# vmingchen/PacBioAssembly

Hardware: AMD Instinct MI355X
Metric: aligned candidate pairs/sec (whole node), 15 kb PacBio reads @15% error (higher is better)
Workload: dtype u32

## Files before the change

### pacbioassembly_amd/csrc/align_bitvec.h

```cpp
#ifndef PBA_ALIGN_BITVEC_H
#define PBA_ALIGN_BITVEC_H

#include <limits.h>

#include <type_traits>

#include "align_rowsweep.h"
#include "dev_common.h"
#include "eq_table.h"
#include "text_ring.h"

#ifndef PBA_BV_EQTAB
#define PBA_BV_EQTAB 1
#endif
#ifndef PBA_BV_RING
#define PBA_BV_RING 1
#endif
#define PBA_BV_EQTAB_NB(nb) (PBA_BV_EQTAB && PBA_BV_RING && (nb) <= 2)

#define PBA_BV_MAX_NB 8
#define PBA_BV_FIN_WORDS(nb) ((2 * (nb) + 1) * 64)
#define PBA_BV_LDS_BYTES(nb) (PBA_BV_EQTAB_NB(nb) ? eqt_lds_words(nb) * 4 : PBA_BV_FIN_WORDS(nb) * 4 + PBA_TXR_BYTES)
#define PBA_BV_BAND_NUM 9
#define PBA_BV_BAND_DEN 16

__device__ __host__ inline int bv_max_span(int nb) { return 2016 * nb + 64; }
__device__ __host__ inline int bv_nb_for_span(int span) {
    const int need = (span - 64 + 2015) / 2016;
    const int nb = need < 1 ? 1 : need;
    return nb <= 4 ? nb : (nb <= 6 ? 6 : (nb <= 8 ? 8 : 0));
}
__device__ __host__ inline int bv_nb_for(int w) { return bv_nb_for_span(2 * w); }

__device__ __forceinline__ uint64_t load_bases32(const uint8_t *seq, int idx) {
    const uint8_t *p = seq + (idx >> 2);
    const uint64_t hi = __builtin_bswap64(ld_u64(p)), nx = __builtin_bswap64(ld_u64(p + 8));
    const int sh = 2 * (idx & 3);
    return sh ? (hi << sh) | (nx >> (64 - sh)) : hi;
}

__device__ __forceinline__ uint32_t compress_even64(uint64_t x) {
    uint32_t lo = (uint32_t)x & 0x55555555u, hi = (uint32_t)(x >> 32) & 0x55555555u;
    lo = (lo | (lo >> 1)) & 0x33333333u; hi = (hi | (hi >> 1)) & 0x33333333u;
    lo = (lo | (lo >> 2)) & 0x0F0F0F0Fu; hi = (hi | (hi >> 2)) & 0x0F0F0F0Fu;
    lo = (lo | (lo >> 4)) & 0x00FF00FFu; hi = (hi | (hi >> 4)) & 0x00FF00FFu;
    lo = (lo | (lo >> 8)) & 0x0000FFFFu; hi = (hi | (hi >> 8)) & 0x0000FFFFu;
    return lo | (hi << 16);
}

__device__ __forceinline__ void load_planes32(const PackedFetch &f, int e, uint32_t &plo, uint32_t &phi) {
    const int idx = f.dir > 0 ? f.org + e : f.org - e - 31;
    const uint32_t *p = f.pl + 2 * (ptrdiff_t)(idx >> 5);
    const uint32_t sh = (uint32_t)idx & 31u;
    const uint32_t lo = __builtin_amdgcn_alignbit(p[2], p[0], sh);
    const uint32_t hi = __builtin_amdgcn_alignbit(p[3], p[1], sh);
    plo = f.dir > 0 ? lo : __builtin_bitreverse32(lo);
    phi = f.dir > 0 ? hi : __builtin_bitreverse32(hi);
}

__device__ __forceinline__ void planes_from_packed(const uint8_t *seq, int idx, uint32_t &plo, uint32_t &phi) {
    const uint64_t x = load_bases32(seq, idx);
    plo = __builtin_bitreverse32(compress_even64(x));
    phi = __builtin_bitreverse32(compress_even64(x >> 1));
}

__device__ __forceinline__ uint32_t addc_mask(uint32_t a, uint32_t b, uint64_t cin, uint64_t &cout) {
    uint32_t d;
    asm("v_addc_co_u32 %0, %1, %2, %3, %4" : "=v"(d), "=s"(cout) : "v"(a), "v"(b), "s"(cin));
    return d;
}

__device__ __forceinline__ uint32_t or_of_and(uint32_t a, uint32_t b, uint32_t c) {
    uint32_t d;
    asm("v_bitop3_b32 %0, %1, %2, %3 bitop3:0xf8" : "=v"(d) : "v"(a), "v"(b), "v"(c));
    return d;
}
__device__ __forceinline__ uint32_t or_of_and_s(uint32_t a, uint32_t b, uint32_t c) {
    uint32_t d;
    asm("v_bitop3_b32 %0, %1, %2, %3 bitop3:0xf8" : "=v"(d) : "v"(a), "v"(b), "s"(c));
    return d;
}
__device__ __forceinline__ uint32_t eq_mask(uint32_t a, uint32_t b, uint32_t c) {
    uint32_t d;
    asm("v_bitop3_b32 %0, %1, %2, %3 bitop3:0x09" : "=v"(d) : "v"(a), "v"(b), "v"(c));
    return d;
}
__device__ __forceinline__ uint64_t bv_uniform64(uint64_t x) {
    return (uint64_t)(uint32_t)__builtin_amdgcn_readfirstlane((int)(uint32_t)x) |
           (uint64_t)(uint32_t)__builtin_amdgcn_readfirstlane((int)(uint32_t)(x >> 32)) << 32;
}
__device__ __forceinline__ uint64_t bv_orn2(uint64_t a, uint64_t b) {
    uint64_t d;
    asm("s_orn2_b64 %0, %1, %2" : "=s"(d) : "s"(a), "s"(b) : "scc");
    return d;
}
__device__ __forceinline__ uint64_t bv_and2(uint64_t a, uint64_t b) {
    uint64_t d;
    asm("s_and_b64 %0, %1, %2" : "=s"(d) : "s"(a), "s"(b) : "scc");
    return d;
}
__device__ __forceinline__ uint32_t bit_mask(uint32_t x, int k) {
    uint32_t d;
    asm("v_bfe_i32 %0, %1, %2, 1" : "=v"(d) : "v"(x), "s"(k));
    return d;
}

#define PBA_BV_CK_WORDS(nb) ((nb) * 128 + 128)
#define PBA_BV_BAIL 0x40000000
template <int NB>
__device__ __forceinline__ void bv_ckpt_store(uint32_t *tr, int tb, int lane, const uint32_t *Pv, const uint32_t *Mv, int s_cur,
                                              uint32_t opened, uint64_t hp_last, uint64_t hn_last) {
    uint32_t *ck = tr + (size_t)((tb - 1) >> 5) * PBA_BV_CK_WORDS(NB);
#pragma unroll
    for (int nb = 0; nb < NB; ++nb) { ck[nb * 128 + lane] = Pv[nb]; ck[nb * 128 + 64 + lane] = Mv[nb]; }
    ck[NB * 128 + lane] = (uint32_t)s_cur | (opened << 31);
    if (lane < 4)
        ck[NB * 128 + 64 + lane] = lane == 0 ? (uint32_t)hp_last : lane == 1 ? (uint32_t)(hp_last >> 32) : lane == 2 ? (uint32_t)hn_last : (uint32_t)(hn_last >> 32);
}

template <int NB, int TRACE = 0, bool BAIL = false, bool RING = false>
__device__ __forceinline__ int bitvec_pass(const PackedFetch &rowsF, int nr, const PackedFetch &colsF, int m, int wleft, int w,
                                           double R, int &best_out, int &besti_out, int &diag_out, uint32_t *fin,
                                           uint32_t *tr = nullptr, bool swap_roles = false, int bail_w = 0) {
    constexpr int RB = 32 * NB;
    const int lane = threadIdx.x & (PBA_WAVE - 1);
    m = __builtin_amdgcn_readfirstlane(m); nr = __builtin_amdgcn_readfirstlane(nr);
    w = __builtin_amdgcn_readfirstlane(w); wleft = __builtin_amdgcn_readfirstlane(wleft);
    const int S = (nr + RB - 1) / RB;
    const int s_m = (m - 1) / RB;
    const int nb_m = ((m - 1) - s_m * RB) >> 5, r_m = (m - 1) & 31;
    const int t1 = m + s_m;
    const int t_end = m + S - 1;
    (void)nb_m; (void)r_m;

    constexpr bool EQT = RING && PBA_BV_EQTAB_NB(NB);
    constexpr int FIN_SB = EQT ? PBA_EQT_LETTERS * NB * PBA_EQT_LANES + PBA_TXR_SLOTS : 2 * NB * PBA_WAVE;
    typedef __attribute__((address_space(3))) uint32_t lds_u32;
    lds_u32 *const tab_lane = (lds_u32 *)fin + lane;
    (void)tab_lane;
#define PBA_BV_FILL_ROWS(sb)                                                          \
    _Pragma("unroll") for (int nb = 0; nb < NB; ++nb) {                               \
        uint32_t plo_, phi_;                                                          \
        load_planes32(rowsF, (sb) * RB + 32 * nb, plo_, phi_);                        \
        tab_lane[(0 * NB + nb) * PBA_EQT_LANES] = ~(plo_ | phi_);                     \
        tab_lane[(1 * NB + nb) * PBA_EQT_LANES] = plo_ & ~phi_;                       \
        tab_lane[(2 * NB + nb) * PBA_EQT_LANES] = ~plo_ & phi_;                       \
        tab_lane[(3 * NB + nb) * PBA_EQT_LANES] = plo_ & phi_;                        \
    }

    uint32_t Pv[NB], Mv[NB], Plo[NB], Phi[NB], acc[NB];
    int s_cur = lane;
    uint32_t opened = 0;
    (void)opened; (void)Plo; (void)Phi;
    if (s_cur < S) {
        if constexpr (EQT) { PBA_BV_FILL_ROWS(s_cur) } else {
#pragma unroll
        for (int nb = 0; nb < NB; ++nb) load_planes32(rowsF, s_cur * RB + 32 * nb, Plo[nb], Phi[nb]);
        }
    }
#pragma unroll
    for (int nb = 0; nb < NB; ++nb) { Pv[nb] = ~0u; Mv[nb] = 0u; acc[nb] = 0u; }

    int T_open = 1, s_op = 0;
    int T_close = min(m, RB + w) + 1, s_cl = 0;
    int T_diag = 1, s_dg = 0;
    int T_seg = min(32, m) + 1, s_sg = 0;
    int s_next = 1;
    (void)T_diag; (void)s_dg;
    constexpr bool LANE_SB = !RING;
#define PBA_BV_LANE_SB() (LANE_SB ? s_cur : s_cl + ((lane - s_cl) & (PBA_WAVE - 1)))
#define PBA_BV_LANE_OPEN() (LANE_SB ? opened != 0 : PBA_BV_LANE_SB() < s_op)
    constexpr bool DIAG_FOLD = !BAIL && NB != 6;
    constexpr int OH_SH = DIAG_FOLD ? 32 : 0;
    typedef typename std::conditional<DIAG_FOLD, uint64_t, uint32_t>::type onehot_t;
    onehot_t one = DIAG_FOLD ? (onehot_t)1 << OH_SH : 0;
    int qd = 0;
    constexpr bool LANE_HOT = BAIL;
    uint32_t dmw = 0;
    (void)dmw; (void)one; (void)qd;

    uint32_t wl = 0, wh = 0;
    typedef __attribute__((address_space(3))) typename std::conditional<EQT, uint32_t, uint64_t>::type txr_cell;
    txr_cell *const ring = (txr_cell *)(fin + (EQT ? PBA_EQT_LETTERS * NB * PBA_EQT_LANES : PBA_BV_FIN_WORDS(NB)));
    const txr_cell *ta = ring;
    (void)wl; (void)wh; (void)ring; (void)ta;
    if constexpr (EQT) {
        static_assert(PBA_TXR_SLOTS <= 3 * PBA_WAVE && PBA_TXR_SLOTS > 2 * PBA_WAVE, "three cells per lane cover the ring");
        ring[lane] = 0; ring[PBA_WAVE + lane] = 0;
        if (lane < PBA_TXR_SLOTS - 2 * PBA_WAVE) ring[2 * PBA_WAVE + lane] = 0;
    }
    int score = 0, fail_row = 0;
    fin[FIN_SB + lane] = 0xFFFFFFFFu;
    uint64_t hp_last = ~0ull, hn_last = 0ull;
    uint64_t live = (S >= PBA_WAVE ? ~0ull : (1ull << S) - 1ull) >> 1;
    uint64_t hpm = ~0ull, hnm = 0ull;

    auto load_text = [&](int tb) {
        if constexpr (RING) {
            const int first = txr_fetch_first(tb, s_cl);
            uint32_t plo, phi;
            load_planes32(colsF, first, plo, phi);
            const int c = lane & (PBA_TXR_CHUNK - 1), slot = txr_slot(first + c), mir = txr_mirror(slot);
            const int dst = (lane >= PBA_TXR_CHUNK && mir >= 0) ? mir : slot;
            if constexpr (EQT) ring[dst] = (((plo >> c) & 1u) | (((phi >> c) & 1u) << 1)) * (uint32_t)(NB * PBA_EQT_LANES * 4);
            else ring[dst] = (uint64_t)(0u - ((plo >> c) & 1u)) | ((uint64_t)(0u - ((phi >> c) & 1u)) << 32);
            ta = ring + txr_addr(tb, PBA_BV_LANE_SB());
        } else {
            load_planes32(colsF, tb - PBA_BV_LANE_SB() - 1, wl, wh);
        }
    };

    auto segment_done = [&](int s, int i) -> int {
        const int rr = i - 1 - s * RB, cnt = (rr & 31) + 1, i0 = i - cnt, q = rr >> 5;
        const int L = s & (PBA_WAVE - 1);
        uint32_t dw = 0;
#pragma unroll
        for (int nb = 0; nb < NB; ++nb) if (q == nb) dw = __builtin_amdgcn_readlane(acc[nb], L);
        dw &= 0xFFFFFFFFu >> (32 - cnt);
        const int end = score + cnt - __builtin_popcount(dw);
        const int ifirst = max(i0 + 1, 11);
        int fr = 0;
        if (i >= ifirst && (double)end > (double)ifirst * R) {
#pragma clang loop unroll(disable) vectorize(disable) interleave(disable)
            for (int k = ifirst - i0; k <= cnt; ++k) {
                const int d = score + k - __builtin_popcount(dw & (0xFFFFFFFFu >> (32 - k)));
                if ((double)d > (double)(i0 + k) * R) { fr = i0 + k; break; }
            }
        }
        if constexpr (BAIL) {
            if (bail_w > 0 && i >= 1024 && fr == 0 &&
                ((float)end - 4.0f * __builtin_sqrtf((float)end)) * (float)m > (float)i * (float)bail_w) fr = PBA_BV_BAIL;
        }
        score = end;
        const bool leaves = rr == RB - 1 && i != m;
        if (lane == L || (DIAG_FOLD && leaves && lane == ((s + 1) & (PBA_WAVE - 1)))) {
#pragma unroll
            for (int nb = 0; nb < NB; ++nb) acc[nb] = 0;
            if constexpr (LANE_HOT) dmw = (i == m || rr == RB - 1) ? 0u : 1u;
        }
        if constexpr (DIAG_FOLD) one = i == m ? 0 : (onehot_t)1 << (leaves ? OH_SH - 1 : OH_SH);
        else one = (i == m || rr == RB - 1) ? 0u : 1u;
        qd = (q + 1) % NB;
        return fr;
    };

#define PBA_BV_EVENTS(DIAG)                                                           \
    {                                                                                 \
        if (DIAG && t == T_seg) {                                                     \
            const int s = s_sg, i = t - 1 - s;                                        \
            seg_fail = segment_done(s, i);                                            \
            if (i == m) T_seg = INT_MAX;                                              \
            else { s_sg = s + (i == s * RB + RB ? 1 : 0); T_seg = min(i + 32, m) + s_sg + 1; } \
        }                                                                             \
        if (t == T_close) {                                                           \
            const int s = s_cl;                                                       \
            if (lane == (s & (PBA_WAVE - 1))) {                                       \
                if (s >= s_m) {               \
                    fin[FIN_SB + lane] = (uint32_t)(LANE_SB ? s_cur : s);  \
                    _Pragma("unroll") for (int nb = 0; nb < NB; ++nb) { fin[2 * nb * PBA_WAVE + lane] = Pv[nb]; fin[(2 * nb + 1) * PBA_WAVE + lane] = Mv[nb]; } \
                }                                                                     \
                                    \
                if constexpr (LANE_SB) { s_cur += PBA_WAVE; opened = 0; }             \
                const int sn = LANE_SB ? s_cur : s + PBA_WAVE;                        \
                 \
                if (s + PBA_WAVE < S) {                                               \
                    if constexpr (EQT) { PBA_BV_FILL_ROWS(sn) } else {                \
                    _Pragma("unroll") for (int nb = 0; nb < NB; ++nb) load_planes32(rowsF, sn * RB + 32 * nb, Plo[nb], Phi[nb]); \
                    }                                                                 \
                }                                                                     \
                if constexpr (RING) ta = ring + txr_addr(t, sn);       \
                else load_text(t - ((t - 1) & 31));                                   \
            }                                                                         \
              \
            if (s + PBA_WAVE < S) {                                                   \
                live |= 1ull << ((s - 1) & (PBA_WAVE - 1));                           \
                hpm = bv_orn2(hp_last, live); hnm = bv_and2(hn_last, live);           \
            }                                                                         \
            live &= ~(1ull << (s & (PBA_WAVE - 1)));                                  \
            s_cl = s + 1;                                                             \
            T_close = s_cl < S ? min(m, s_cl * RB + RB + w) + s_cl + 1 : INT_MAX;     \
        }                                                                             \
        if (t == T_open) {                                                            \
            if (lane == (s_op & (PBA_WAVE - 1))) {                                    \
                _Pragma("unroll") for (int nb = 0; nb < NB; ++nb) { Pv[nb] = ~0u; Mv[nb] = 0u; } \
                if constexpr (LANE_SB) opened = 1;                                    \
            }                                                                         \
            s_op += 1;                                                                \
            T_open = s_op < S ? max(1, s_op * RB + 1 - wleft) + s_op : INT_MAX;       \
        }                                                                             \
        if constexpr (!DIAG_FOLD) {                                                   \
            if (DIAG && t == T_diag) {                                                \
                if (lane == (s_dg & (PBA_WAVE - 1))) {                                \
                    _Pragma("unroll") for (int nb = 0; nb < NB; ++nb) acc[nb] = 0;    \
                    if constexpr (LANE_HOT) dmw = 1u;                                 \
                }                                                                     \
                one = 1u; qd = 0;                                                     \
                s_dg += 1;                                                            \
                T_diag = s_dg * RB < m ? s_dg * (RB + 1) + 1 : INT_MAX;               \
            }                                                                         \
        }                                                                             \
        s_next = min(T_open, T_close);                                                \
        if (DIAG) s_next = min(s_next, DIAG_FOLD ? T_seg : min(T_seg, T_diag));       \
        if constexpr (TRACE == 1) st_on = ((__builtin_amdgcn_ballot_w64(PBA_BV_LANE_OPEN()) >> (lane & 48)) & 0xFFFFull) != 0; \
    }

#define PBA_BV_HIN()                                                                  \
    uint64_t hp = (hpm << 1) | (hpm >> 63);                                           \
    uint64_t hn = (hnm << 1) | (hnm >> 63);
#define PBA_BV_HOUT()                                                                 \
    hp_last = hp; hn_last = hn;                                                       \
    hpm = bv_orn2(hp, live); hnm = bv_and2(hn, live);

#define PBA_BV_BLOCK(nb, PH_PRE, MH_PRE, D0, EQ)                                     \
    {                                                                                \
        const uint32_t Eq = EQT ? eqr[nb] : eq_mask(Plo[nb] ^ clo, Phi[nb], chi);    \
        EQ = Eq;                                                                     \
        const uint32_t pv = Pv[nb], mv = Mv[nb];                                     \
        uint64_t unused;                                                             \
        const uint32_t sum = addc_mask(Eq & pv, pv, hn, unused);    \
        const uint32_t Xh = (sum ^ pv) | Eq;                                         \
        const uint32_t Ph = mv | ~(Xh | pv);                                         \
        const uint32_t Mh = pv & Xh;                                                 \
        D0 = Xh | mv;                                                                \
        PH_PRE = Ph; MH_PRE = Mh;                                                    \
        const uint32_t Ph2 = addc_mask(Ph, Ph, hp, hp);                              \
        const uint32_t Mh2 = addc_mask(Mh, Mh, hn, hn);                              \
        Pv[nb] = Mh2 | ~(D0 | Ph2);                                                  \
        Mv[nb] = Ph2 & D0;                                                           \
    }

    uint2 *const tr_lane = (uint2 *)tr + lane;
    (void)tr_lane;
    bool st_on = false;
    (void)st_on;
#define PBA_BV_TRP() (tr_lane + (size_t)(t - 1) * (NB * 64))
#define PBA_BV_TEXT(OFS)                                                             \
        uint32_t clo = 0, chi = 0, eqr[NB];                                          \
        _Pragma("unroll") for (int nb = 0; nb < NB; ++nb) eqr[nb] = eqn[OFS][nb];    \
        (void)clo; (void)chi; (void)eqr;                                             \
        if constexpr (EQT) { }                                                       \
        else if constexpr (RING) { const uint64_t cell = ta[OFS]; clo = (uint32_t)cell; chi = (uint32_t)(cell >> 32); } \
        else { clo = bit_mask(wl, k + (OFS)); chi = bit_mask(wh, k + (OFS)); }
#define PBA_BV_ROWS(OFS)                                                             \
        {                                                                            \
        const lds_u32 *const row = (const lds_u32 *)((const __attribute__((address_space(3))) uint8_t *)tab_lane + cq[OFS]); \
        _Pragma("unroll") for (int nb = 0; nb < NB; ++nb) eqn[OFS][nb] = row[nb * PBA_EQT_LANES]; \
        }
#define PBA_BV_STEP1(QD, OFS)                                                        \
        {                                                                            \
        const int t = tb + k + (OFS);                                                \
        (void)t;                                                                     \
        PBA_BV_TEXT(OFS)                                                             \
        PBA_BV_HIN();                                                                \
        _Pragma("unroll")                                                            \
        for (int nb = 0; nb < NB; ++nb) {                                            \
            uint32_t d0, php, mhp, eq;                                               \
            PBA_BV_BLOCK(nb, php, mhp, d0, eq);                                      \
            (void)php; (void)mhp; (void)eq;                                          \
            if constexpr (TRACE == 1) {       \
                if (st_on)                    \
                    PBA_BV_TRP()[nb * 64] = make_uint2(eq | ~d0, swap_roles ? Pv[nb] : php); \
            }                                                                        \
                               \
            if constexpr (LANE_HOT) acc[nb] = or_of_and(acc[nb], d0, dmw); else       \
            if ((QD) < 0 || nb == (QD)) acc[nb] = or_of_and_s(acc[nb], d0, (uint32_t)(oh >> OH_SH)); \
        }                                                                            \
        PBA_BV_HOUT()                                                                \
                                               \
        if constexpr (LANE_HOT) asm("v_add_u32 %0, %1, %1" : "=v"(dmw) : "v"(dmw)); else oh <<= 1; \
        }
#define PBA_BV_STRETCH1(QD)                                                          \
        uint32_t cq[2] = {0u, 0u}, eqn[2][NB] = {};                                  \
        (void)cq; (void)eqn;                                                         \
        if constexpr (EQT) {                                                         \
            if ((kstop - k) & 1) { cq[0] = ta[0]; PBA_BV_ROWS(0) PBA_BV_STEP1(QD, 0) ta += 1; k += 1; } \
            while (k < kstop) {                                                      \
                cq[0] = ta[0]; cq[1] = ta[1];                                        \
                PBA_BV_ROWS(0) PBA_BV_ROWS(1)                                        \
                PBA_BV_STEP1(QD, 0)                                                  \
                _Pragma("unroll") for (int nb = 0; nb < NB; ++nb) asm("" : "+v"(Pv[nb]), "+v"(Mv[nb])); \
                PBA_BV_STEP1(QD, 1)                                                  \
                ta += 2; k += 2;                                                     \
            }                                                                        \
        } else if constexpr (RING) {                                                 \
            if ((kstop - k) & 1) { PBA_BV_STEP1(QD, 0) ta += 1; k += 1; }            \
            while (k < kstop) {                                                      \
                PBA_BV_STEP1(QD, 0)                                                  \
                 \
                _Pragma("unroll") for (int nb = 0; nb < NB; ++nb) asm("" : "+v"(Pv[nb]), "+v"(Mv[nb])); \
                PBA_BV_STEP1(QD, 1)                                                  \
                ta += 2; k += 2;                                                     \
            }                                                                        \
        } else {                                                                     \
            do { PBA_BV_STEP1(QD, 0) } while (++k < kstop);                          \
        }
    for (int tbv = 1; tbv <= t1; tbv += 32) {
        const int tb = __builtin_amdgcn_readfirstlane(tbv);
        if constexpr (TRACE == 2) bv_ckpt_store<NB>(tr, tb, lane, Pv, Mv, PBA_BV_LANE_SB(), LANE_SB ? opened : (PBA_BV_LANE_OPEN() ? 1u : 0u), hp_last, hn_last);
        load_text(tb);
        if (fail_row) break;
        int kend = min(32, t1 - tb + 1);
        for (int k = 0; k < kend;) {
        if (tb + k == s_next) {
            const int t = tb + k;
            int seg_fail = 0;
            PBA_BV_EVENTS(true);
            if (seg_fail) { fail_row = seg_fail; kend = k + 1; }
        }
        const int kstop = min(kend, s_next - tb);
        onehot_t oh = 0;
        if constexpr (DIAG_FOLD) oh = (onehot_t)bv_uniform64(one);
        else if constexpr (!LANE_HOT) oh = __builtin_amdgcn_readfirstlane(one);
        if constexpr (NB == 2 && TRACE != 1 && !LANE_HOT) {
            if (__builtin_amdgcn_readfirstlane(qd) == 0) { PBA_BV_STRETCH1(0); } else { PBA_BV_STRETCH1(1); }
        } else {
            PBA_BV_STRETCH1(NB == 1 ? 0 : -1);
        }
        if constexpr (!LANE_HOT) one = oh;
        }
    }
    if (fail_row == 0) fail_row = segment_done(s_m, m);
    if (fail_row) return __builtin_amdgcn_readfirstlane(fail_row);
    s_next = min(T_open, T_close);
    hpm = bv_orn2(hp_last, live); hnm = bv_and2(hn_last, live);

    for (int tb = t1 + 1; tb <= t_end;) {
        const int k0 = (tb - 1) & 31;
        if (k0 == 0) {
            if constexpr (TRACE == 2) bv_ckpt_store<NB>(tr, tb, lane, Pv, Mv, PBA_BV_LANE_SB(), LANE_SB ? opened : (PBA_BV_LANE_OPEN() ? 1u : 0u), hp_last, hn_last);
            load_text(tb);
        }
        const int kend = min(32, k0 + (t_end - tb + 1));
        const int tc = tb - k0;
        for (int k = k0; k < kend;) {
        if (tc + k == s_next) {
            const int t = tc + k;
            int seg_fail = 0;
            (void)seg_fail;
            PBA_BV_EVENTS(false);
        }
        const int kstop = min(kend, s_next - tc);
        do {
        const int t = tc + k;
        (void)t;
        uint32_t cq[1] = {0u}, eqn[1][NB] = {};
        (void)cq; (void)eqn;
        if constexpr (EQT) { cq[0] = ta[0]; PBA_BV_ROWS(0) }
        PBA_BV_TEXT(0)
        PBA_BV_HIN();
#pragma unroll
        for (int nb = 0; nb < NB; ++nb) {
            uint32_t d0, php, mhp, eq;
            PBA_BV_BLOCK(nb, php, mhp, d0, eq);
            (void)d0; (void)eq; (void)php; (void)mhp;
            if constexpr (TRACE == 1) {
                if (st_on)
                    PBA_BV_TRP()[nb * 64] = make_uint2(eq | ~d0, swap_roles ? Pv[nb] : php);
            }
        }
        PBA_BV_HOUT()
        if constexpr (RING) ta += 1;
        } while (++k < kstop);
        }
        tb += kend - k0;
    }
#undef PBA_BV_STRETCH1
#undef PBA_BV_STEP1
#undef PBA_BV_ROWS
#undef PBA_BV_TEXT
#undef PBA_BV_FILL_ROWS
#undef PBA_BV_BLOCK
#undef PBA_BV_TRP
#undef PBA_BV_HOUT
#undef PBA_BV_HIN
#undef PBA_BV_EVENTS
    if (const int sb = PBA_BV_LANE_SB(); PBA_BV_LANE_OPEN() && sb >= s_m && sb < S) {
        fin[FIN_SB + lane] = (uint32_t)sb;
#pragma unroll
        for (int nb = 0; nb < NB; ++nb) { fin[2 * nb * PBA_WAVE + lane] = Pv[nb]; fin[(2 * nb + 1) * PBA_WAVE + lane] = Mv[nb]; }
    }
#undef PBA_BV_LANE_OPEN
#undef PBA_BV_LANE_SB
    const int fin_s = (int)fin[FIN_SB + lane];
    int b_tot[NB], b_min[NB], b_pos[NB];
#pragma unroll
    for (int nb = 0; nb < NB; ++nb) {
        const int row0 = fin_s * RB + nb * 32;
        const uint32_t fpv = fin_s >= 0 ? fin[2 * nb * PBA_WAVE + lane] : 0u, fmv = fin_s >= 0 ? fin[(2 * nb + 1) * PBA_WAVE + lane] : 0u;
        int v = 0, pm = INT_MAX, pp = 0;
        for (int r = 0; r < 32; ++r) {
            const int row = row0 + r + 1;
            if (fin_s >= 0 && row > m && row <= nr) {
                v += (int)((fpv >> r) & 1u) - (int)((fmv >> r) & 1u);
                if (v < pm) { pm = v; pp = r; }
            }
        }
        b_tot[nb] = v; b_min[nb] = pm; b_pos[nb] = pp;
    }
    int gbest = __builtin_amdgcn_readfirstlane(score), gi = m, run = gbest;
    diag_out = gbest;
    for (int sb = s_m; sb < S; ++sb) {
        const int L = sb & (PBA_WAVE - 1);
#pragma unroll
        for (int nb = 0; nb < NB; ++nb) {
            const int pm = __builtin_amdgcn_readlane(b_min[nb], L);
            if (pm != INT_MAX && run + pm < gbest) {
                gbest = run + pm;
                gi = sb * RB + nb * 32 + __builtin_amdgcn_readlane(b_pos[nb], L) + 1;
            }
            run += __builtin_amdgcn_readlane(b_tot[nb], L);
        }
    }
    best_out = gbest;
    besti_out = gi;
    return 0;
}

__device__ __host__ inline int bv_full_wl(int md) { return md / 2 + 1 < md ? md / 2 + 1 : md; }
__device__ __host__ inline bool bitvec_supports(int max_dst) { return bv_nb_for_span(bv_full_wl(max_dst) + max_dst) != 0; }
__device__ __host__ inline int bv_first_w(int md) {
    const int w = (md / 2 > (int)((long long)md * PBA_BV_BAND_NUM / PBA_BV_BAND_DEN)
                       ? md / 2 : (int)((long long)md * PBA_BV_BAND_NUM / PBA_BV_BAND_DEN)) + 1;
    return w > md ? md : w;
}
__device__ __host__ inline int bv_first_wl(int md) {
    const int wl = bv_first_w(md) / 2 + 1;
    return wl > md ? md : wl;
}
__device__ __host__ inline int bv_pass1_w(int md, int nb) {
    int w = bv_first_w(md);
    const int room = (bv_max_span(nb) - 4) * 2 / 3;
    if (room > w) w = room;
    return w > md ? md : w;
}
__device__ __host__ inline int bv_pass1_wl(int md, int nb) {
    const int wl = bv_pass1_w(md, nb) / 2 + 1;
    return wl > md ? md : wl;
}
__device__ __forceinline__ bool bv_fail_certified(int fr, double R, int wl, int md) {
    return 2 * wl + 2 > md || (double)fr * R < (double)(2 * wl + 2);
}
__device__ __forceinline__ bool bv_goal_certified(int best, int wl, int w, int md) {
    return (w >= md && 2 * wl + 1 >= md) || (best <= w && best <= 2 * wl + 1);
}

#define PBA_RC_UNCERTIFIED (-3)

#ifndef PBA_BV_RING
#define PBA_BV_RING 1
#endif
template <int NB, bool BAIL = false>
__device__ __forceinline__ void align_bitvec(const PackedFetch &fa, int la, const PackedFetch &fb, int lb, double R,
                                             int maxn, int maxm, bool full_band, uint16_t *lds, int lds_cells,
                                             AlnOut &o, bool need_diag = false) {
    aln_params(la, lb, R, o);
    const int len_a = o.len_a, len_b = o.len_b, md = o.max_dst;
    if (maxn > 0 && (len_a >= maxn + maxm || md >= maxm)) return;
    const bool a_rows = len_a > len_b;
    const int m = a_rows ? len_b : len_a, n = a_rows ? len_a : len_b;
    if (m <= 10) {
        align_rowsweep(fa, la, fb, lb, R, maxn, maxm, lds, lds_cells, o);
        return;
    }
    const int w = full_band ? md : bv_pass1_w(md, NB), wl = full_band ? bv_full_wl(md) : bv_pass1_wl(md, NB);
    if (wl + w > bv_max_span(NB)) { o.rc = -2; return; }
    const PackedFetch rowsF = a_rows ? fa : fb, colsF = a_rows ? fb : fa;
    int best = 0, besti = 0, diag = 0;
    const int bail_w = (BAIL && !full_band && w < md) ? w : 0;
    const int fr = bitvec_pass<NB, 0, BAIL, PBA_BV_RING && !BAIL>(rowsF, min(n, m + w), colsF, m, w, wl, R, best, besti, diag, (uint32_t *)lds, nullptr, false, bail_w);
    if (fr) {
        bool gave_up = false;
        if constexpr (BAIL) gave_up = fr == PBA_BV_BAIL;
        if (!gave_up && bv_fail_certified(fr, R, wl, md)) o.fail_row = fr; else o.rc = PBA_RC_UNCERTIFIED;
        return;
    }
    if (!bv_goal_certified(best, wl, w, md)) { o.rc = PBA_RC_UNCERTIFIED; return; }
    const bool diag_ok = bv_goal_certified(diag, wl, w, md);
    if (need_diag && !diag_ok) { o.rc = PBA_RC_UNCERTIFIED; return; }
    o.cost = best;
    o.diag = diag_ok ? diag : -1;
    o.matlen_a = a_rows ? besti : m;
    o.matlen_b = a_rows ? m : besti;
    o.rc = ((double)o.matlen_b < (double)len_b * (1.0 - R)) ? -1 : o.matlen_b;
}

#endif
```

Baseline: 20.19 million.

## Shift band state down one lane on segment close instead of rotating lanes

For the EQ-table ring path, closing a segment now shifts Pv/Mv/acc down one lane with DPP, so lane 0 always holds the oldest open segment. This removes the live-mask orn/and work and the rotate in the per-column horizontal carry, which becomes a plain scalar shift. The cost is a special non-rotated step on close columns, DPP moves on every close, and column-indexed LDS addressing. The new mapping touches event handling, the ring addressing and the final readout, so it carries correctness risk.

```diff
diff --git a/pacbioassembly_amd/csrc/align_bitvec.h b/pacbioassembly_amd/csrc/align_bitvec.h
--- a/pacbioassembly_amd/csrc/align_bitvec.h
+++ b/pacbioassembly_amd/csrc/align_bitvec.h
@@ -8,6 +8,7 @@
 #include "align_rowsweep.h"
 #include "dev_common.h"
 #include "eq_table.h"
+#include "lane_shift.h"
 #include "text_ring.h"
 
 #ifndef PBA_BV_EQTAB
@@ -17,6 +18,9 @@
 #define PBA_BV_RING 1
 #endif
 #define PBA_BV_EQTAB_NB(nb) (PBA_BV_EQTAB && PBA_BV_RING && (nb) <= 2)
+#ifndef PBA_BV_SHIFT
+#define PBA_BV_SHIFT 1
+#endif
 
 #define PBA_BV_MAX_NB 8
 #define PBA_BV_FIN_WORDS(nb) ((2 * (nb) + 1) * 64)
@@ -98,6 +102,19 @@
     uint64_t d;
     asm("s_and_b64 %0, %1, %2" : "=s"(d) : "s"(a), "s"(b) : "scc");
     return d;
+}
+__device__ __forceinline__ uint64_t bv_shl1(uint64_t a) {
+    uint64_t d;
+    asm("s_lshl_b64 %0, %1, 1" : "=s"(d) : "s"(a) : "scc");
+    return d;
+}
+__device__ __forceinline__ uint64_t bv_shl1_or1(uint64_t a) {
+    uint64_t d;
+    asm("s_lshl_b64 %0, %1, 1\n\ts_or_b64 %0, %0, 1" : "=&s"(d) : "s"(a) : "scc");
+    return d;
+}
+__device__ __forceinline__ uint32_t bv_lane_below(uint32_t x) {
+    return (uint32_t)__builtin_amdgcn_update_dpp((int)x, (int)x, 0x130 , 0xf, 0xf, false);
 }
 __device__ __forceinline__ uint32_t bit_mask(uint32_t x, int k) {
     uint32_t d;
@@ -136,8 +153,8 @@
     constexpr bool EQT = RING && PBA_BV_EQTAB_NB(NB);
     constexpr int FIN_SB = EQT ? PBA_EQT_LETTERS * NB * PBA_EQT_LANES + PBA_TXR_SLOTS : 2 * NB * PBA_WAVE;
     typedef __attribute__((address_space(3))) uint32_t lds_u32;
-    lds_u32 *const tab_lane = (lds_u32 *)fin + lane;
-    (void)tab_lane;
+    constexpr bool SHIFT = EQT && PBA_BV_SHIFT;
+#define tab_lane ((lds_u32 *)fin + (SHIFT ? lsh_col(lane, s_cl) : lane))
 #define PBA_BV_FILL_ROWS(sb)                                                          \
     _Pragma("unroll") for (int nb = 0; nb < NB; ++nb) {                               \
         uint32_t plo_, phi_;                                                          \
@@ -153,6 +170,8 @@
     uint32_t opened = 0;
     (void)opened; (void)Plo; (void)Phi;
     if (s_cur < S) {
+        constexpr int s_cl = 0;
+        (void)s_cl;
         if constexpr (EQT) { PBA_BV_FILL_ROWS(s_cur) } else {
 #pragma unroll
         for (int nb = 0; nb < NB; ++nb) load_planes32(rowsF, s_cur * RB + 32 * nb, Plo[nb], Phi[nb]);
@@ -168,7 +187,8 @@
     int s_next = 1;
     (void)T_diag; (void)s_dg;
     constexpr bool LANE_SB = !RING;
-#define PBA_BV_LANE_SB() (LANE_SB ? s_cur : s_cl + ((lane - s_cl) & (PBA_WAVE - 1)))
+#define PBA_BV_LANE_SB() (LANE_SB ? s_cur : SHIFT ? lsh_sb(lane, s_cl) : s_cl + ((lane - s_cl) & (PBA_WAVE - 1)))
+#define PBA_BV_LANE_OF(s) (SHIFT ? lsh_lane(s, s_cl) : (s) & (PBA_WAVE - 1))
 #define PBA_BV_LANE_OPEN() (LANE_SB ? opened != 0 : PBA_BV_LANE_SB() < s_op)
     constexpr bool DIAG_FOLD = !BAIL && NB != 6;
     constexpr int OH_SH = DIAG_FOLD ? 32 : 0;
@@ -212,7 +232,7 @@
 
     auto segment_done = [&](int s, int i) -> int {
         const int rr = i - 1 - s * RB, cnt = (rr & 31) + 1, i0 = i - cnt, q = rr >> 5;
-        const int L = s & (PBA_WAVE - 1);
+        const int L = PBA_BV_LANE_OF(s);
         uint32_t dw = 0;
 #pragma unroll
         for (int nb = 0; nb < NB; ++nb) if (q == nb) dw = __builtin_amdgcn_readlane(acc[nb], L);
@@ -233,7 +253,7 @@
         }
         score = end;
         const bool leaves = rr == RB - 1 && i != m;
-        if (lane == L || (DIAG_FOLD && leaves && lane == ((s + 1) & (PBA_WAVE - 1)))) {
+        if (lane == L || (DIAG_FOLD && leaves && lane == PBA_BV_LANE_OF(s + 1))) {
 #pragma unroll
             for (int nb = 0; nb < NB; ++nb) acc[nb] = 0;
             if constexpr (LANE_HOT) dmw = (i == m || rr == RB - 1) ? 0u : 1u;
@@ -254,6 +274,22 @@
         }                                                                             \
         if (t == T_close) {                                                           \
             const int s = s_cl;                                                       \
+            if constexpr (SHIFT) {                                                    \
+                 \
+                if (lane == 0 && s >= s_m) {                                        \
+                    tab_lane[FIN_SB] = (uint32_t)s;                                   \
+                    _Pragma("unroll") for (int nb = 0; nb < NB; ++nb) { tab_lane[2 * nb * PBA_WAVE] = Pv[nb]; tab_lane[(2 * nb + 1) * PBA_WAVE] = Mv[nb]; } \
+                }                                                                     \
+                _Pragma("unroll") for (int nb = 0; nb < NB; ++nb) {                   \
+                    Pv[nb] = bv_lane_below(Pv[nb]); \
+                    Mv[nb] = bv_lane_below(Mv[nb]); \
+                    acc[nb] = bv_lane_below(acc[nb]); \
+                }                                                                     \
+                s_cl = s + 1;                 \
+                if (lane == PBA_WAVE - 1 && s + PBA_WAVE < S) { PBA_BV_FILL_ROWS(s + PBA_WAVE) } \
+                ta = ring + lsh_ring_addr(t, lane, s_cl);                             \
+                closed = true;                \
+            } else {                                                                \
             if (lane == (s & (PBA_WAVE - 1))) {                                       \
                 if (s >= s_m) {               \
                     fin[FIN_SB + lane] = (uint32_t)(LANE_SB ? s_cur : s);  \
@@ -277,11 +313,12 @@
                 hpm = bv_orn2(hp_last, live); hnm = bv_and2(hn_last, live);           \
             }                                                                         \
             live &= ~(1ull << (s & (PBA_WAVE - 1)));                                  \
+            }                                                                         \
             s_cl = s + 1;                                                             \
             T_close = s_cl < S ? min(m, s_cl * RB + RB + w) + s_cl + 1 : INT_MAX;     \
         }                                                                             \
         if (t == T_open) {                                                            \
-            if (lane == (s_op & (PBA_WAVE - 1))) {                                    \
+            if (lane == PBA_BV_LANE_OF(s_op)) {                                       \
                 _Pragma("unroll") for (int nb = 0; nb < NB; ++nb) { Pv[nb] = ~0u; Mv[nb] = 0u; } \
                 if constexpr (LANE_SB) opened = 1;                                    \
             }                                                                         \
@@ -304,12 +341,14 @@
         if constexpr (TRACE == 1) st_on = ((__builtin_amdgcn_ballot_w64(PBA_BV_LANE_OPEN()) >> (lane & 48)) & 0xFFFFull) != 0; \
     }
 
-#define PBA_BV_HIN()                                                                  \
-    uint64_t hp = (hpm << 1) | (hpm >> 63);                                           \
-    uint64_t hn = (hnm << 1) | (hnm >> 63);
+#define PBA_BV_HIN(CLOSED)                                                            \
+    uint64_t hp = SHIFT ? ((CLOSED) ? hpm : bv_shl1_or1(hpm)) : (hpm << 1) | (hpm >> 63); \
+    uint64_t hn = SHIFT ? ((CLOSED) ? hnm : bv_shl1(hnm)) : (hnm << 1) | (hnm >> 63);
 #define PBA_BV_HOUT()                                                                 \
+    if constexpr (SHIFT) { hpm = hp; hnm = hn; } else {                               \
     hp_last = hp; hn_last = hn;                                                       \
-    hpm = bv_orn2(hp, live); hnm = bv_and2(hn, live);
+    hpm = bv_orn2(hp, live); hnm = bv_and2(hn, live);                                 \
+    }
 
 #define PBA_BV_BLOCK(nb, PH_PRE, MH_PRE, D0, EQ)                                     \
     {                                                                                \
@@ -346,12 +385,13 @@
         const lds_u32 *const row = (const lds_u32 *)((const __attribute__((address_space(3))) uint8_t *)tab_lane + cq[OFS]); \
         _Pragma("unroll") for (int nb = 0; nb < NB; ++nb) eqn[OFS][nb] = row[nb * PBA_EQT_LANES]; \
         }
-#define PBA_BV_STEP1(QD, OFS)                                                        \
+#define PBA_BV_STEP1(QD, OFS) PBA_BV_STEP1X(QD, OFS, false)
+#define PBA_BV_STEP1X(QD, OFS, CLOSED)                                               \
         {                                                                            \
         const int t = tb + k + (OFS);                                                \
         (void)t;                                                                     \
         PBA_BV_TEXT(OFS)                                                             \
-        PBA_BV_HIN();                                                                \
+        PBA_BV_HIN(CLOSED);                                                              \
         _Pragma("unroll")                                                            \
         for (int nb = 0; nb < NB; ++nb) {                                            \
             uint32_t d0, php, mhp, eq;                                               \
@@ -401,11 +441,24 @@
         if (fail_row) break;
         int kend = min(32, t1 - tb + 1);
         for (int k = 0; k < kend;) {
+        bool closed = false;
+        (void)closed;
         if (tb + k == s_next) {
             const int t = tb + k;
             int seg_fail = 0;
             PBA_BV_EVENTS(true);
             if (seg_fail) { fail_row = seg_fail; kend = k + 1; }
+        }
+        if constexpr (SHIFT) {
+            if (closed) {
+                onehot_t oh = (onehot_t)bv_uniform64(one);
+                uint32_t cq[1] = {ta[0]}, eqn[1][NB];
+                PBA_BV_ROWS(0)
+                PBA_BV_STEP1X(NB == 1 ? 0 : -1, 0, true)
+                one = oh;
+                ta += 1; k += 1;
+                continue;
+            }
         }
         const int kstop = min(kend, s_next - tb);
         onehot_t oh = 0;
@@ -422,7 +475,8 @@
     if (fail_row == 0) fail_row = segment_done(s_m, m);
     if (fail_row) return __builtin_amdgcn_readfirstlane(fail_row);
     s_next = min(T_open, T_close);
-    hpm = bv_orn2(hp_last, live); hnm = bv_and2(hn_last, live);
+    if constexpr (SHIFT) { hpm = bv_uniform64(hpm); hnm = bv_uniform64(hnm); }
+    else { hpm = bv_orn2(hp_last, live); hnm = bv_and2(hn_last, live); }
 
     for (int tb = t1 + 1; tb <= t_end;) {
         const int k0 = (tb - 1) & 31;
@@ -433,38 +487,47 @@
         const int kend = min(32, k0 + (t_end - tb + 1));
         const int tc = tb - k0;
         for (int k = k0; k < kend;) {
+        bool closed = false;
+        (void)closed;
         if (tc + k == s_next) {
             const int t = tc + k;
             int seg_fail = 0;
             (void)seg_fail;
             PBA_BV_EVENTS(false);
         }
+#define PBA_BV_STEP2(CLOSED)                                                          \
+        {                                                                             \
+        const int t = tc + k;                                                         \
+        (void)t;                                                                      \
+        uint32_t cq[1] = {0u}, eqn[1][NB] = {};                                       \
+        (void)cq; (void)eqn;                                                          \
+        if constexpr (EQT) { cq[0] = ta[0]; PBA_BV_ROWS(0) }                          \
+        PBA_BV_TEXT(0)                                                                \
+        PBA_BV_HIN(CLOSED);                                                           \
+        _Pragma("unroll")                                                             \
+        for (int nb = 0; nb < NB; ++nb) {                                             \
+            uint32_t d0, php, mhp, eq;                                                \
+            PBA_BV_BLOCK(nb, php, mhp, d0, eq);                                       \
+            (void)d0; (void)eq; (void)php; (void)mhp;                                 \
+            if constexpr (TRACE == 1) {       \
+                if (st_on)                    \
+                    PBA_BV_TRP()[nb * 64] = make_uint2(eq | ~d0, swap_roles ? Pv[nb] : php); \
+            }                                                                         \
+        }                                                                             \
+        PBA_BV_HOUT()                                                                 \
+        if constexpr (RING) ta += 1;                                                  \
+        }
+        if constexpr (SHIFT) {
+            if (closed) { PBA_BV_STEP2(true) k += 1; continue; }
+        }
         const int kstop = min(kend, s_next - tc);
-        do {
-        const int t = tc + k;
-        (void)t;
-        uint32_t cq[1] = {0u}, eqn[1][NB] = {};
-        (void)cq; (void)eqn;
-        if constexpr (EQT) { cq[0] = ta[0]; PBA_BV_ROWS(0) }
-        PBA_BV_TEXT(0)
-        PBA_BV_HIN();
-#pragma unroll
-        for (int nb = 0; nb < NB; ++nb) {
-            uint32_t d0, php, mhp, eq;
-            PBA_BV_BLOCK(nb, php, mhp, d0, eq);
-            (void)d0; (void)eq; (void)php; (void)mhp;
-            if constexpr (TRACE == 1) {
-                if (st_on)
-                    PBA_BV_TRP()[nb * 64] = make_uint2(eq | ~d0, swap_roles ? Pv[nb] : php);
-            }
-        }
-        PBA_BV_HOUT()
-        if constexpr (RING) ta += 1;
-        } while (++k < kstop);
+        do { PBA_BV_STEP2(false) } while (++k < kstop);
         }
         tb += kend - k0;
     }
 #undef PBA_BV_STRETCH1
+#undef PBA_BV_STEP2
+#undef PBA_BV_STEP1X
 #undef PBA_BV_STEP1
 #undef PBA_BV_ROWS
 #undef PBA_BV_TEXT
@@ -475,12 +538,15 @@
 #undef PBA_BV_HIN
 #undef PBA_BV_EVENTS
     if (const int sb = PBA_BV_LANE_SB(); PBA_BV_LANE_OPEN() && sb >= s_m && sb < S) {
-        fin[FIN_SB + lane] = (uint32_t)sb;
-#pragma unroll
-        for (int nb = 0; nb < NB; ++nb) { fin[2 * nb * PBA_WAVE + lane] = Pv[nb]; fin[(2 * nb + 1) * PBA_WAVE + lane] = Mv[nb]; }
+        const int col = SHIFT ? lsh_col(lane, s_cl) : lane;
+        fin[FIN_SB + col] = (uint32_t)sb;
+#pragma unroll
+        for (int nb = 0; nb < NB; ++nb) { fin[2 * nb * PBA_WAVE + col] = Pv[nb]; fin[(2 * nb + 1) * PBA_WAVE + col] = Mv[nb]; }
     }
 #undef PBA_BV_LANE_OPEN
 #undef PBA_BV_LANE_SB
+#undef PBA_BV_LANE_OF
+#undef tab_lane
     const int fin_s = (int)fin[FIN_SB + lane];
     int b_tot[NB], b_min[NB], b_pos[NB];
 #pragma unroll
diff --git a/pacbioassembly_amd/csrc/lane_shift.h b/pacbioassembly_amd/csrc/lane_shift.h
--- /dev/null
+++ b/pacbioassembly_amd/csrc/lane_shift.h
@@ -0,0 +1,21 @@
+#ifndef PBA_LANE_SHIFT_H
+#define PBA_LANE_SHIFT_H
+
+#include <stdint.h>
+
+#include "eq_table.h"
+
+#define PBA_LSH_LANES 64
+
+PBA_TXR_FN int lsh_sb(int lane, int s_cl) { return s_cl + lane; }
+PBA_TXR_FN int lsh_lane(int s, int s_cl) { return s - s_cl; }
+PBA_TXR_FN int lsh_col(int lane, int s_cl) { return (lane + s_cl) & (PBA_LSH_LANES - 1); }
+PBA_TXR_FN int lsh_src_lane(int lane) { return (lane + 1) & (PBA_LSH_LANES - 1); }
+PBA_TXR_FN uint64_t lsh_hin_plus(uint64_t hpm) { return (hpm << 1) | 1ull; }
+PBA_TXR_FN uint64_t lsh_hin_minus(uint64_t hnm) { return hnm << 1; }
+PBA_TXR_FN uint64_t lsh_hin_plus_closed(uint64_t hpm) { return hpm; }
+PBA_TXR_FN uint64_t lsh_hin_minus_closed(uint64_t hnm) { return hnm; }
+PBA_TXR_FN int lsh_ring_addr(int t, int lane, int s_cl) { return txr_addr(t, lsh_sb(lane, s_cl)); }
+PBA_TXR_FN int lsh_read_word(int cell, int b, int lane, int s_cl) { return eqt_read_word(cell, b, lsh_col(lane, s_cl)); }
+
+#endif
```

Result: faster. 21.39 million (median of 6 runs) (+5.9%).
